# ORNL/DDStore

Hardware: NVIDIA H100
Metric: batch_fetch_GBps (higher is better)
Workload: dtype u8

## Files before the change

ddstore_b200/csrc/kernels.cu:

```cuda
#include <cuda_runtime.h>
#include <stdint.h>
#include <stdio.h>
#include <stdlib.h>
#include <string.h>

#include <algorithm>
#include <atomic>
#include <type_traits>

#include "kernels.h"

namespace {

thread_local char g_cuda_err[512] = "";
std::atomic<unsigned long long> g_launches{0};

#define CUDA_TRY(expr)                                                                                   \
    do {                                                                                                 \
        cudaError_t e__ = (expr);                                                                        \
        if (e__ != cudaSuccess) {                                                                        \
            snprintf(g_cuda_err, sizeof(g_cuda_err), "%s failed: %s (%s:%d)", #expr, cudaGetErrorString(e__), \
                     __FILE__, __LINE__);                                                                \
            return (int)e__ ? (int)e__ : -1;                                                             \
        }                                                                                                \
// ... 176 lines not shown
            start[k] = e.x;
            count[k] = e.y;
        }
    } else if (p.ids) {
        int64_t id[K];
#pragma unroll
        for (int k = 0; k < K; k++) {
            live[k] = idx[k] < limit;
            id[k] = live[k] ? p.ids[idx[k]] : 0;
            vp[k] = &var;
        }
#pragma unroll
        for (int k = 0; k < K; k++) {
            badid[k] = live[k] && (id[k] < 0 || id[k] >= p.nsamples);
            const bool ok = live[k] && !badid[k];
            const longlong2 e = ok ? ldg_pair(&p.tab[id[k]]) : make_longlong2(0, 0);
            start[k] = e.x;
            count[k] = e.y;
        }
    } else {
#pragma unroll
        for (int k = 0; k < K; k++) {
            live[k] = idx[k] < limit;
            badid[k] = false;
            start[k] = live[k] ? p.starts[idx[k]] : 0;
            count[k] = live[k] ? p.counts[idx[k]] : 0;
            vp[k] = &var;
        }
    }
#pragma unroll
    for (int k = 0; k < K; k++) {
        src[k] = 0;
        nbytes[k] = 0;
        if (!live[k]) continue;
        if (badid[k]) {
            report(status, tag, idx[k], DDSK_CODE_SAMPLE);
            continue;
        }
        uint64_t s = 0;
        const int code = dev_locate(*vp[k], start[k], count[k], &s);
        if (code) {
            report(status, tag, idx[k], code);
            continue;
        }
        src[k] = s;
        nbytes[k] = count[k] * vp[k]->row_bytes;
    }
}

__device__ __forceinline__ int64_t warp_incl_scan(int64_t v, int lane) {
#pragma unroll
    for (int d = 1; d < 32; d <<= 1) {
        int64_t o = __shfl_up_sync(0xffffffffu, v, d);
        if (lane >= d) v += o;
    }
    return v;
}
__device__ __forceinline__ int64_t warp_sum(int64_t v) {
#pragma unroll
    for (int d = 16; d > 0; d >>= 1) v += __shfl_xor_sync(0xffffffffu, v, d);
    return v;
}

struct GatherArgs {
    ddsk_var_t var;
    const int64_t *starts;
    int64_t count;
    const uint64_t *req_src;
    const int64_t *req_dst;
    const uint32_t *seg_tab;
    PlanSrc plan;
    int64_t *total_out;
    int64_t nreq;
    char *dst;
    int64_t dst_cap;
    int64_t *offsets_out;
    unsigned long long *status;
    unsigned long long status_tag;
    unsigned int *counters;
    char *mdst[DDSK_MAX_MULTI];
    int64_t mcap[DDSK_MAX_MULTI];
    int64_t *moffsets[DDSK_MAX_MULTI];
    int min_seg_chunks;
    int overlap, skip_wait;
    int wait1_valid, wait2_valid;
    unsigned int seq;
    unsigned int *ovl;
    int wait_plan;
    unsigned long long *plan_word;
    int64_t plan_tiles;
    unsigned int *tickets;
    unsigned long long *host_mirror;
    unsigned long long *dbg;
    const ddsk_push_t *push;
    int64_t push_nreq;
    unsigned long long push_step;
};

constexpr int64_t SEG_GRAIN = 16384;

struct Piece {
    uint64_t src;
    int64_t dpos;
    uint32_t n;
    uint32_t off;
};

template <int PCAP>
struct PlanView {
    uint32_t src_s, dst_s;
    __device__ __forceinline__ uint64_t s(int64_t i) const { return lds64(src_s + (uint32_t)i * 8u); }
    __device__ __forceinline__ int64_t d(int64_t i) const { return (int64_t)lds32(dst_s + (uint32_t)i * 4u); }
};
template <>
struct PlanView<0> {
    const uint64_t *src;
    const int64_t *dst;
    const uint32_t *seg_tab;
    __device__ __forceinline__ uint64_t s(int64_t i) const { return __ldcg(&src[i]); }
    __device__ __forceinline__ int64_t d(int64_t i) const { return __ldcg(&dst[i]); }
};

template <bool FIXED, int CH, int PCAP, bool VALIGN = false>
struct ChunkWalker {
    int64_t seg_pos = 0, seg_end = 0, T = 0, seg_bytes = 0, nseg = 0, nb = 0;
    int64_t gwarp = 0, nwarps = 1;
    bool first_claim = true, static_claims = false;
    int64_t cur_seg = 0;
    unsigned int pend = 0;
    bool armed = false;
    bool gate_ok = true;
    int64_t r = 0, win_base = -64;
    int64_t nreq = 0;
    int push_n = 0, push_me = 0, push_par = 0;
    const int64_t *push_rbase = nullptr;
    const uint64_t *push_win = nullptr;
    int64_t push_idx_off = 0;
    PlanView<PCAP> pv;
    bool valign = false;
    int64_t vb[VALIGN ? DDSK_MAX_MULTI : 1];
    uint64_t w_src = 0;
    int64_t w_dst = 0, w_n = 0;

    __device__ __forceinline__ void load_window(const GatherArgs &a, int lane) {
        win_base = r;
        int64_t idx = r + lane;
        w_src = 0;
        w_dst = 0;
        w_n = 0;
        if (idx < nreq) {
            if (FIXED && push_n > 0) {
                int p = 0;
                for (int k = 1; k < push_n; k++)
                    if (idx >= push_rbase[k]) p = k;
                const int64_t i = idx - push_rbase[p];
                const int64_t start = ld_relaxed_sys_s64((const int64_t *)(push_win[p] + push_idx_off) + i);
                uint64_t s = 0;
                int owner = 0;
                const int code = dev_locate_owner(a.var, start, a.count, &s, &owner);
                if (code && owner == push_me) {
                    unsigned long long *st = (unsigned long long *)push_win[p] + 3;
                    asm volatile("red.relaxed.sys.global.min.u64 [%0], %1;" ::"l"(st), "l"(((unsigned long long)i << 8) | (unsigned long long)code) : "memory");
                }
                w_src = (code || owner != push_me) ? 0 : s;
                w_dst = idx * nb;
                w_n = nb;
            } else if (FIXED) {
                uint64_t s = 0;
                int code = dev_locate(a.var, a.starts[idx], a.count, &s);
                if (code) report(a.status, a.status_tag, idx, code);
                w_src = code ? 0 : s;
                w_dst = idx * nb;
                w_n = nb;
            } else {
                w_src = pv.s(idx);
                w_dst = pv.d(idx);
                w_n = pv.d(idx + 1) - w_dst;
            }
        }
    }

    __device__ __forceinline__ int64_t align_to_var(int64_t pos) const {
        int64_t b = vb[0];
#pragma unroll
        for (int k = 1; k < (VALIGN ? DDSK_MAX_MULTI : 1); k++)
            if (pos >= vb[k]) b = vb[k];
        return b + ((pos - b) & ~(int64_t)7);
    }

    __device__ __forceinline__ int64_t locate_var(const GatherArgs &a, int64_t pos, int lane) {
        if constexpr (VALIGN && PCAP == 0) {
            if (valign) {
                int64_t r0 = (int64_t)__ldcg(&a.seg_tab[(pos + 7) / SEG_GRAIN]);
                while (r0 > 0 && pv.d(r0) > pos) r0--;
                return r0;
            }
        }
        if (PCAP == 0) {
            int64_t r0 = (int64_t)__ldcg(&a.seg_tab[pos / SEG_GRAIN]);
            return r0;
        }
        int64_t lo = 0, hi = nreq;
        while (hi - lo > 1) {
            int64_t step = (hi - lo + 31) / 32;
            int64_t idx = lo + (int64_t)(lane + 1) * step;
            bool le = (idx < hi) && (pv.d(idx) <= pos);
            int k = __popc(__ballot_sync(0xffffffffu, le));
            lo = lo + (int64_t)k * step;
            hi = min(hi, lo + step);
        }
        return lo;
    }

    __device__ __forceinline__ void arm(const GatherArgs &a, int lane) {
        if (lane == 0) pend = atomicAdd(a.tickets, 1u);
        armed = true;
    }

    template <int STAGE, typename Gate>
    __device__ __forceinline__ uint32_t next_group(const GatherArgs &a, int lane, Piece &pc, Gate &&gate) {
        while (true) {
            if (seg_pos >= seg_end) {
                int64_t seg;
                if (first_claim) {
                    first_claim = false;
                    seg = gwarp;
                    if (!static_claims && seg < nseg && gate_ok) arm(a, lane);
                } else if (static_claims) {
                    seg = cur_seg + nwarps;
                } else {
                    if (!armed) {
                        gate();
                        gate_ok = true;
                        arm(a, lane);
                    }
                    seg = nwarps + (int64_t)__shfl_sync(0xffffffffu, pend, 0);
                    armed = false;
                    if (seg < nseg) arm(a, lane);
                }
                cur_seg = seg;
                if (seg >= nseg) return 0;
                seg_pos = seg * seg_bytes;
                seg_end = min(T, seg_pos + seg_bytes);
                if constexpr (VALIGN) {
                    if (valign) {
                        seg_pos = align_to_var(seg_pos);
                        if (seg_end < T) seg_end = align_to_var(seg_end);
                        if (seg_pos >= seg_end) continue;
                    }
                }
                r = FIXED ? seg_pos / nb : locate_var(a, seg_pos, lane);
            }
            if (r >= nreq) {
                seg_pos = seg_end;
                continue;
            }
            if (r < win_base || r >= win_base + 32) load_window(a, lane);
            {
                const int wl = (int)(r - win_base);
                const uint64_t s0 = __shfl_sync(0xffffffffu, w_src, wl);
                const int64_t d0 = __shfl_sync(0xffffffffu, w_dst, wl);
                const int64_t e0 = d0 + __shfl_sync(0xffffffffu, w_n, wl);
                const int64_t p0 = max(d0, seg_pos);
                const int64_t len = min(min(e0, seg_end) - p0, (int64_t)CH);
                if (len >= CH / 2 || p0 + len < e0) {
                    seg_pos = p0 + len;
                    if (seg_pos >= e0) r++;
                    if (s0 == 0) continue;
                    const uint64_t src = s0 + (uint64_t)(p0 - d0);
                    pc.src = lane == 0 ? src : 0;
                    pc.dpos = p0;
                    pc.n = lane == 0 ? (uint32_t)len : 0u;
                    pc.off = 0;
                    return ((uint32_t)(src & 15u) + (uint32_t)len + 15u) & ~15u;
                }
            }
            const int srcl = (int)(r - win_base) + lane;
            const uint64_t q_src = __shfl_sync(0xffffffffu, w_src, srcl & 31);
            const int64_t q_d0 = __shfl_sync(0xffffffffu, w_dst, srcl & 31);
            const int64_t q_n = __shfl_sync(0xffffffffu, w_n, srcl & 31);
            const int64_t q_end = q_d0 + q_n;
            const bool valid = srcl < 32 && r + lane < nreq && q_d0 < seg_end;
            const int64_t p0 = max(q_d0, seg_pos);
            int64_t len = min(q_end, seg_end) - p0;
            len = max(len, (int64_t)0);
            len = min(len, (int64_t)CH);
            const bool complete = p0 + len >= q_end;
            const bool copy = valid && len > 0 && q_src != 0;
            const uint64_t src = q_src + (uint64_t)(p0 - q_d0);
            const uint32_t sz = copy ? (((uint32_t)(src & 15u) + (uint32_t)len + 15u) & ~15u) : 0u;
            uint32_t end = sz;
#pragma unroll
            for (int d = 1; d < 32; d <<= 1) {
                uint32_t o = __shfl_up_sync(0xffffffffu, end, d);
                if (lane >= d) end += o;
            }
            const unsigned ok = __ballot_sync(0xffffffffu, valid && end <= (uint32_t)STAGE);
            const unsigned part = __ballot_sync(0xffffffffu, valid && !complete);
            int m = ok == 0xffffffffu ? 32 : __ffs(~ok) - 1;
            if (part) m = min(m, __ffs(part));
            const bool active = lane < m;
            const int64_t new_pos = __shfl_sync(0xffffffffu, p0 + len, m - 1);
            const uint32_t total = __shfl_sync(0xffffffffu, end, m - 1);
            r += __popc(__ballot_sync(0xffffffffu, active && complete));
            seg_pos = max(seg_pos, new_pos);
            if (total == 0) continue;
            pc.src = (active && copy) ? src : 0;
            pc.dpos = p0;
            pc.n = (active && copy) ? (uint32_t)len : 0u;
            pc.off = end - sz;
            return total;
        }
    }
};

template <int WS, bool BYTES>
__device__ __forceinline__ void rephase_loop(uint32_t sbase, char *dv, uint32_t nv, uint32_t bs8, int lane) {
#pragma unroll 4
    for (uint32_t j = (uint32_t)lane; j < nv; j += 32) {
        const uint4 lo = lds128(sbase + (j << 4));
        const uint4 hi = lds128(sbase + (j << 4) + 16);
        const uint32_t w[8] = {lo.x, lo.y, lo.z, lo.w, hi.x, hi.y, hi.z, hi.w};
        uint4 out;
        if (BYTES) {
            out.x = __funnelshift_r(w[WS + 0], w[WS + 1], bs8);
            out.y = __funnelshift_r(w[WS + 1], w[WS + 2], bs8);
// ... 172 lines not shown
        const uint32_t k = head + nv * E + (uint32_t)lane;
        cvt_one<CODE>(s0 + (k << IL), d + ((size_t)k << OL), lut);
    }
}

struct NoCvt {
    int32_t unused_;
};
template <bool CVT>
using CvtParam = typename std::conditional<CVT, ddsk_cvt_t, NoCvt>::type;

template <int NW, int PCAP, bool CVT = false>
__device__ __forceinline__ int64_t plan_in_smem(const GatherArgs &a, const PlanView<PCAP> &pv, int64_t *wtot, int warp,
                                                int lane, bool writer, int code = 0) {
    auto out = [&](int64_t x) -> int64_t {
        if constexpr (CVT) return cvt_scale(x, code);
        else return x;
    };
    const int64_t nreq = a.nreq;
    const int64_t per_warp = ((nreq + NW * 128 - 1) / (NW * 128)) * 128;
    const int64_t w0 = min(nreq, (int64_t)warp * per_warp), w1 = min(nreq, w0 + per_warp);
    int64_t lane_sum = 0;
    for (int64_t b = w0; b < w1; b += 128) {
        int64_t idx[4], nb[4];
        uint64_t sv[4];
#pragma unroll
        for (int k = 0; k < 4; k++) idx[k] = b + k * 32 + lane;
        plan_many<4>(a.var, a.plan, idx, w1, a.status, a.status_tag, sv, nb);
#pragma unroll
        for (int k = 0; k < 4; k++) {
            if (idx[k] < w1) {
                sts64(pv.src_s + (uint32_t)idx[k] * 8u, sv[k]);
                sts32(pv.dst_s + (uint32_t)idx[k] * 4u, (uint32_t)min(nb[k], (int64_t)0xFFFFFFFFll));
                lane_sum += nb[k];
            }
        }
    }
    const int64_t wsum = warp_sum(lane_sum);
    if (lane == 0) wtot[warp] = wsum;
    __syncthreads();
    int64_t mine = lane < NW ? wtot[lane] : 0;
    const int64_t T = warp_sum(mine);
    const int64_t base = warp_sum(lane < warp ? mine : 0);
    int64_t run = base;
    for (int64_t b = w0; b < w1; b += 32) {
        const int64_t i = b + lane;
        const int64_t v = i < w1 ? (int64_t)lds32(pv.dst_s + (uint32_t)i * 4u) : 0;
        const int64_t incl = warp_incl_scan(v, lane);
        if (i < w1) {
            sts32(pv.dst_s + (uint32_t)i * 4u, (uint32_t)(run + incl - v));
            if (writer && a.offsets_out) a.offsets_out[i] = out(run + incl - v);
        }
        run += __shfl_sync(0xffffffffu, incl, 31);
    }
    if (warp == 0 && lane == 0) {
        sts32(pv.dst_s + (uint32_t)nreq * 4u, (uint32_t)min(T, (int64_t)0xFFFFFFFFll));
        if (writer) {
            if (a.offsets_out) a.offsets_out[nreq] = out(T);
            if (a.total_out) *a.total_out = T;
        }
    }
    __syncthreads();
    return T;
}

struct PieceDesc {
    int64_t dpos;
    uint32_t n, pack;
};

__device__ __forceinline__ void spin_until_done(const unsigned int *ovl, unsigned int q, unsigned long long *status,
                                                unsigned long long tag, int64_t nreq) {
    const uint64_t t0 = globaltimer_ns();
    while ((int)(ld_acquire_u32(&ovl[4 + (q & 3u)]) - q) < 0) {
        __nanosleep(100);
        if (globaltimer_ns() - t0 > 4000000000ull) {
            report(status, tag, nreq, DDSK_CODE_WATCHDOG);
            __trap();
        }
    }
}

template <bool FIXED, int NW, int S, int CH, int PCAP, bool CVT = false>
__global__ void __launch_bounds__(NW * 32, 1) dds_gather_kernel(const __grid_constant__ GatherArgs a,
                                                                const __grid_constant__ CvtParam<CVT> c) {
    constexpr int STAGE = CH + 32;
    constexpr bool PUSH = FIXED && !CVT;
    extern __shared__ __align__(128) unsigned char smem_dyn[];
    __shared__ __align__(8) uint64_t full_bar[NW][S];
    __shared__ __align__(16) PieceDesc desc[NW][S][32];
    __shared__ int64_t wtot[PCAP > 0 ? NW : 1];
    __shared__ int64_t push_rbase[PUSH ? DDSK_MAX_RANKS + 1 : 1];
    __shared__ uint64_t push_win[PUSH ? DDSK_MAX_RANKS : 1];

    const int lane = threadIdx.x & 31;
    const int warp = threadIdx.x >> 5;
    const int64_t gwarp = (int64_t)blockIdx.x * NW + warp;
    const int64_t nwarps = (int64_t)gridDim.x * NW;

    if (lane == 0) {
#pragma unroll
        for (int s = 0; s < S; s++) mbar_init(smem_u32(&full_bar[warp][s]), 1);
        fence_mbar_init();
    }
    uint32_t lut_s = 0;
    if constexpr (CVT) {
        lut_s = smem_u32(smem_dyn) + (uint32_t)(NW * S * STAGE + (PCAP ? PCAP * 12 + 16 : 0));
        for (int i = threadIdx.x; i < c.lut_bytes / 4; i += NW * 32) sts32(lut_s + 4u * (uint32_t)i, c.lut[i]);
        __syncthreads();
    }
    int code0 = 0;
    if constexpr (CVT) code0 = c.code[0];
    if (a.dbg && threadIdx.x == 0) a.dbg[blockIdx.x * 4 + 0] = globaltimer_ns();
    if (a.overlap && !a.wait1_valid) {
        asm volatile("griddepcontrol.wait;" ::: "memory");
        asm volatile("griddepcontrol.launch_dependents;" ::: "memory");
    } else {
        asm volatile("griddepcontrol.launch_dependents;" ::: "memory");
        if (!a.skip_wait) asm volatile("griddepcontrol.wait;" ::: "memory");
    }
    bool gate_open = !(a.overlap && a.wait2_valid);
    auto pass_gate = [&]() {
        if (!gate_open) {
            if (lane == 0) spin_until_done(a.ovl, a.seq - 2u, a.status, a.status_tag, a.nreq);
            __syncwarp();
            gate_open = true;
        }
    };

    ChunkWalker<FIXED, CH, PCAP, CVT> w;
    if (!FIXED) {
        if constexpr (PCAP > 0) {
            w.pv.src_s = smem_u32(smem_dyn) + (uint32_t)(NW * S * STAGE);
            w.pv.dst_s = w.pv.src_s + (uint32_t)PCAP * 8u;
            const bool writer = blockIdx.x == 0;
            if (writer) pass_gate();
            w.T = plan_in_smem<NW, PCAP, CVT>(a, w.pv, wtot, warp, lane, writer, code0);
        } else {
            w.pv.src = a.req_src;
            w.pv.dst = a.req_dst;
            w.pv.seg_tab = a.seg_tab;
            if (a.wait_plan) {
                const bool need_gate = !gate_open;
                unsigned long long pw = 0;
                const uint64_t t0 = globaltimer_ns();
                while (true) {
                    bool ok = true;
                    if (lane == 0) {
                        pw = ld_acquire_u64(&a.plan_word[a.seq & 3u]);
                        ok = (pw >> 40) == (unsigned long long)a.plan_tiles;
                    } else if (lane == 1 && need_gate) {
                        ok = (int)(ld_acquire_u32(&a.ovl[4 + ((a.seq - 2u) & 3u)]) - (a.seq - 2u)) >= 0;
                    }
                    if (__all_sync(0xffffffffu, ok)) break;
                    __nanosleep(100);
                    if (globaltimer_ns() - t0 > 4000000000ull) {
                        report(a.status, a.status_tag, a.nreq, DDSK_CODE_WATCHDOG);
                        __trap();
                    }
                }
                gate_open = true;
                w.T = (int64_t)(__shfl_sync(0xffffffffu, pw, 0) & 0xFFFFFFFFFFull);
            } else {
                w.T = __ldcg(&a.req_dst[a.nreq]);
            }
        }
    }

    const bool push = PUSH && a.push != nullptr;
    if (FIXED && push) {
        const ddsk_push_t *ps = a.push;
        const int P = ps->nranks, me = ps->me, par = (int)(a.push_step & 1ull);
        if (blockIdx.x == 0 && threadIdx.x == 0) {
            unsigned long long *hdr = (unsigned long long *)ps->win[me];
            *(volatile unsigned long long *)&hdr[1 + par] = (unsigned long long)a.push_nreq;
            __threadfence_system();
            st_release_sys_u64(&hdr[0], a.push_step);
        }
        const uint64_t t0 = globaltimer_ns();
        for (int r0 = 0; r0 < P; r0 += 32) {
            const int r = r0 + lane;
            while (r < P && ld_acquire_sys_u64((const unsigned long long *)ps->win[r]) < a.push_step) {
                __nanosleep(200);
                if (globaltimer_ns() - t0 > 30000000000ull) {
                    report(a.status, a.status_tag, a.nreq, DDSK_CODE_WATCHDOG);
                    __trap();
                }
            }
        }
        __syncwarp();
        if (warp == 0) {
            int64_t n = 0;
            for (int r0 = 0; r0 < P; r0 += 32) {
                const int r = r0 + lane;
                int64_t mine_n = 0;
                if (r < P) {
                    push_win[r] = (uint64_t)ps->win[r];
                    mine_n = ld_relaxed_sys_s64((const int64_t *)ps->win[r] + 1 + par);
                }
                const int64_t incl = warp_incl_scan(mine_n, lane);
                if (r < P) push_rbase[r] = n + incl - mine_n;
                n += __shfl_sync(0xffffffffu, incl, 31);
            }
            if (lane == 0) push_rbase[P] = n;
        }
        __syncthreads();
        w.push_n = P;
        w.push_me = me;
        w.push_par = par;
        w.push_rbase = push_rbase;
        w.push_win = push_win;
        w.push_idx_off = ps->idx_off[par];
    }
    if (a.dbg && threadIdx.x == 0) a.dbg[blockIdx.x * 4 + 1] = globaltimer_ns();
    bool dbg_first = a.dbg != nullptr && warp == 0;
    w.gwarp = gwarp;
    w.nwarps = nwarps;
    w.static_claims = a.tickets == nullptr;
    w.gate_ok = gate_open;
    w.nb = (FIXED && a.count <= a.var.lenlist[a.var.nranks - 1]) ? a.count * a.var.row_bytes : 0;
    w.nreq = (FIXED && push) ? push_rbase[w.push_n] : a.nreq;
    if (FIXED) w.T = w.nb * w.nreq;
    bool over = w.T > a.dst_cap;
    const int64_t push_dst_off = (FIXED && push) ? a.push->dst_off[w.push_par] : 0;
    const bool multi = !FIXED && a.plan.nvars > 1;
    int64_t vbase[DDSK_MAX_MULTI + 1];
#pragma unroll
    for (int v = 0; v <= DDSK_MAX_MULTI; v++) vbase[v] = INT64_MAX;
    if (multi) {
        over = false;
#pragma unroll
        for (int v = 0; v < DDSK_MAX_MULTI; v++)
            if (v < a.plan.nvars) vbase[v] = w.pv.d((int64_t)v * a.plan.per_var);
#pragma unroll
        for (int v = 0; v < DDSK_MAX_MULTI; v++)
            if (v < a.plan.nvars) {
                const int64_t endv = v + 1 < a.plan.nvars ? vbase[v + 1] : w.T;
                over |= endv - vbase[v] > a.mcap[v];
            }
        if (PCAP > 0) over |= w.T > 0xFFFFFFFFll;
        if constexpr (CVT) {
            w.valign = true;
#pragma unroll
            for (int v = 0; v < DDSK_MAX_MULTI; v++) w.vb[v] = vbase[v];
        }
    }
    auto dst_of = [&](int64_t dpos) -> char * {
        if (FIXED && push) {
            int p = 0;
            for (int k = 1; k < w.push_n; k++)
                if (dpos >= push_rbase[k] * w.nb) p = k;
            return (char *)push_win[p] + push_dst_off + (dpos - push_rbase[p] * w.nb);
        }
        if (!multi) return a.dst + dpos;
        int64_t b = vbase[0];
        char *d = a.mdst[0];
#pragma unroll
        for (int k = 1; k < DDSK_MAX_MULTI; k++)
            if (dpos >= vbase[k]) {
                b = vbase[k];
                d = a.mdst[k];
            }
        return d + (dpos - b);
    };
    auto out_of = [&](int64_t dpos, int &code, uint32_t &lut) -> char * {
        if constexpr (CVT) {
            if (!multi) {
                code = code0;
                lut = lut_s + (uint32_t)c.lut_off[0];
                return a.dst + cvt_scale(dpos, code0);
            }
            int64_t b = vbase[0];
            char *d = a.mdst[0];
            int cd = c.code[0], lo = c.lut_off[0];
#pragma unroll
            for (int k = 1; k < DDSK_MAX_MULTI; k++)
                if (dpos >= vbase[k]) {
                    b = vbase[k];
                    d = a.mdst[k];
                    cd = c.code[k];
                    lo = c.lut_off[k];
                }
            code = cd;
            lut = lut_s + (uint32_t)lo;
            return d + cvt_scale(dpos - b, cd);
        } else {
            return nullptr;
        }
    };
    {
        int64_t target = w.T / (nwarps * 8);
        const int64_t unit = (!FIXED && PCAP == 0) ? SEG_GRAIN : (int64_t)CH;
        target = max((int64_t)a.min_seg_chunks * CH, min(target, (int64_t)1 << 20));
        target = max(target, unit);
        if (FIXED && w.nb > 0 && w.nb <= target)
            w.seg_bytes = (target / w.nb) * w.nb;
        else
            w.seg_bytes = (target / unit) * unit;
        w.nseg = w.T > 0 ? (w.T + w.seg_bytes - 1) / w.seg_bytes : 0;
    }
    if (over) {
        if (gwarp == 0 && lane == 0) report(a.status, a.status_tag, a.nreq, DDSK_CODE_CAPACITY);
        w.nseg = 0;
    }

    if (FIXED && !push && (w.nb <= 0 || over)) {
        for (int64_t i = gwarp * 32 + lane; i < a.nreq; i += nwarps * 32) {
            uint64_t s;
            int code = dev_locate(a.var, a.starts[i], a.count, &s);
            if (code) report(a.status, a.status_tag, i, code);
        }
    }

    const uint32_t ring = smem_u32(smem_dyn) + (uint32_t)warp * (uint32_t)(S * STAGE);

    uint32_t issued = 0, consumed = 0;
    bool more = w.nseg > 0;
    while (true) {
        while (more && issued - consumed < (uint32_t)(S - 1)) {
            Piece pc;
            const uint32_t total = w.template next_group<STAGE>(a, lane, pc, pass_gate);
            if (total == 0) {
                more = false;
                break;
            }
            const uint32_t st = issued % S;
            const uint32_t bar = smem_u32(&full_bar[warp][st]);
            bulk_wait_read<1>();
            if (lane == 0) mbar_expect_tx(bar, total);
            __syncwarp();
            const uint32_t al = (uint32_t)(pc.src & 15u);
            desc[warp][st][lane].dpos = pc.dpos;
            desc[warp][st][lane].n = pc.n;
            desc[warp][st][lane].pack = pc.off | (al << 16);
            if (pc.n)
                tma_load_1d(ring + st * STAGE + pc.off, (const void *)(pc.src - al), (al + pc.n + 15u) & ~15u, bar);
            issued++;
        }
        if (consumed == issued) break;
        const uint32_t st = consumed % S;
        const uint32_t parity = (consumed / S) & 1u;
        const uint32_t bar = smem_u32(&full_bar[warp][st]);
        if (!mbar_try_wait(bar, parity)) {
            const uint64_t t0 = globaltimer_ns();
            while (!mbar_try_wait(bar, parity)) {
                if (globaltimer_ns() - t0 > 4000000000ull) {
                    report(a.status, a.status_tag, a.nreq, DDSK_CODE_WATCHDOG);
                    __trap();
                }
            }
        }
        __syncwarp();
        if (dbg_first) {
            dbg_first = false;
            if (lane == 0) a.dbg[blockIdx.x * 4 + 2] = globaltimer_ns();
        }
        pass_gate();
        if (!w.static_claims && !w.gate_ok) {
            w.gate_ok = true;
            if (!w.armed) w.arm(a, lane);
        }
        const int64_t my_dpos = desc[warp][st][lane].dpos;
        const uint32_t my_n = desc[warp][st][lane].n;
        const uint32_t my_pack = desc[warp][st][lane].pack;
        if constexpr (CVT) {
            int my_code;
            uint32_t my_lut;
            char *const my_dst = out_of(my_dpos, my_code, my_lut);
            const bool direct = my_code == 0 && my_n != 0 && (((uint32_t)(uint64_t)my_dst | my_n | (my_pack >> 16)) & 15u) == 0;
            if (direct) tma_store_1d(my_dst, ring + st * STAGE + (my_pack & 0xffffu), my_n);
            unsigned todo = __ballot_sync(0xffffffffu, my_n != 0 && !direct);
            while (todo) {
                const int j = __ffs(todo) - 1;
                todo &= todo - 1;
                const int64_t dpos = __shfl_sync(0xffffffffu, my_dpos, j);
                const uint32_t n = __shfl_sync(0xffffffffu, my_n, j);
                const uint32_t pk = __shfl_sync(0xffffffffu, my_pack, j);
                int code;
                uint32_t lut;
                char *const d = out_of(dpos, code, lut);
                const uint32_t s0 = ring + st * STAGE + (pk & 0xffffu);
                switch (code) {
                case DDSK_CVT_F32_BF16: cvt_drain<DDSK_CVT_F32_BF16>(s0 + (pk >> 16), d, n, lut, lane); break;
                case DDSK_CVT_F32_F16: cvt_drain<DDSK_CVT_F32_F16>(s0 + (pk >> 16), d, n, lut, lane); break;
                case DDSK_CVT_F64_F32: cvt_drain<DDSK_CVT_F64_F32>(s0 + (pk >> 16), d, n, lut, lane); break;
                case DDSK_CVT_U8_LUT16: cvt_drain<DDSK_CVT_U8_LUT16>(s0 + (pk >> 16), d, n, lut, lane); break;
                case DDSK_CVT_U8_LUT32: cvt_drain<DDSK_CVT_U8_LUT32>(s0 + (pk >> 16), d, n, lut, lane); break;
                default: drain_chunk<CH>(s0, pk >> 16, d, n, lane); break;
                }
            }
        } else {
        char *const my_dst = dst_of(my_dpos);
        const bool direct = my_n != 0 && (((uint32_t)(uint64_t)my_dst | my_n | (my_pack >> 16)) & 15u) == 0;
        if (direct) tma_store_1d(my_dst, ring + st * STAGE + (my_pack & 0xffffu), my_n);
        unsigned todo = __ballot_sync(0xffffffffu, my_n != 0 && !direct);
        while (todo) {
            const int j = __ffs(todo) - 1;
            todo &= todo - 1;
            const int64_t dpos = __shfl_sync(0xffffffffu, my_dpos, j);
            const uint32_t n = __shfl_sync(0xffffffffu, my_n, j);
            const uint32_t pk = __shfl_sync(0xffffffffu, my_pack, j);
            drain_chunk<CH>(ring + st * STAGE + (pk & 0xffffu), pk >> 16, dst_of(dpos), n, lane);
        }
        }
        bulk_commit();
        __syncwarp();
        consumed++;
    }
    if (a.overlap || (FIXED && push)) {
        bulk_wait_all<0>();
        fence_proxy_async_global();
    } else {
        bulk_wait_read<0>();
    }
    __syncwarp();
    pass_gate();
    if (multi) {
        for (int64_t i = gwarp * 32 + lane; i < a.nreq + a.plan.nvars; i += nwarps * 32) {
            const int v = (int)(i / (a.plan.per_var + 1));
            const int64_t j = i - (int64_t)v * (a.plan.per_var + 1);
            if (v < a.plan.nvars && a.moffsets[v]) {
                const int64_t basev = w.pv.d((int64_t)v * a.plan.per_var);
                int64_t e = (v * a.plan.per_var + j == a.nreq) ? w.T : w.pv.d((int64_t)v * a.plan.per_var + j);
                if constexpr (CVT) a.moffsets[v][j] = cvt_scale(e - basev, c.code[v]);
                else a.moffsets[v][j] = e - basev;
            }
        }
        if constexpr (CVT) {
            if (gwarp == 0 && lane == 0 && a.total_out) {
                int64_t t = 0;
#pragma unroll
                for (int v = 0; v < DDSK_MAX_MULTI; v++)
                    if (v < a.plan.nvars) t += cvt_scale((v + 1 < a.plan.nvars ? vbase[v + 1] : w.T) - vbase[v], c.code[v]);
                *a.total_out = t;
            }
        }
    }
    if (FIXED && a.offsets_out && !push) {
        if constexpr (CVT) {
            for (int64_t i = gwarp * 32 + lane; i <= a.nreq; i += nwarps * 32) a.offsets_out[i] = cvt_scale(i * w.nb, code0);
        } else {
            for (int64_t i = gwarp * 32 + lane; i <= a.nreq; i += nwarps * 32) a.offsets_out[i] = i * w.nb;
        }
// ... 260 lines not shown
        __syncthreads();
        const int state = sh_state;
        const unsigned long long q = req[0];
        if (state != 0) {
            if (threadIdx.x == 0) {
                if (state == 2) {
                    *(volatile unsigned long long *)&mb->resp = (q << 8);
                    __threadfence_system();
                }
                *(volatile unsigned long long *)&mb->exit_gen = gen;
                __threadfence_system();
            }
            return;
        }
        const int64_t start = (int64_t)req[1], count = (int64_t)req[2], cap = (int64_t)req[4];
        char *dp = (char *)req[3];
        const ddsk_var_t &var = vars[(int)(req[5] & 0xFFFFFFFFull)];
        uint64_t src = 0;
        const int code = dev_locate(var, start, count, &src);
        const int64_t n = code ? 0 : count * var.row_bytes;
        unsigned long long st = 0;
        if (code) st = (unsigned long long)code;
        else if (n > cap) st = DDSK_CODE_CAPACITY;
        if (st == 0 && n > 0) {
            const char *sp = (const char *)src;
            if ((((uint64_t)sp | (uint64_t)dp | (uint64_t)n) & 15u) == 0) {
                for (int64_t i = threadIdx.x; i < (n >> 4); i += blockDim.x) ((uint4 *)dp)[i] = ((const uint4 *)sp)[i];
            } else if ((((uint64_t)sp | (uint64_t)dp | (uint64_t)n) & 3u) == 0) {
                for (int64_t i = threadIdx.x; i < (n >> 2); i += blockDim.x) ((uint32_t *)dp)[i] = ((const uint32_t *)sp)[i];
            } else {
                for (int64_t i = threadIdx.x; i < n; i += blockDim.x) dp[i] = sp[i];
            }
            __threadfence_system();
        }
        __syncthreads();
        if (threadIdx.x == 0) *(volatile unsigned long long *)&mb->resp = (q << 8) | st;
        served = q;
    }
}

__global__ void dds_touch_kernel(const uint4 *__restrict__ p, size_t n, unsigned int *sink) {
    unsigned int acc = 0;
    for (size_t i = (size_t)blockIdx.x * blockDim.x + threadIdx.x; i < n; i += (size_t)gridDim.x * blockDim.x) {
        const uint4 v = p[i];
        acc ^= v.x ^ v.y ^ v.z ^ v.w;
    }
    if (acc == 0x9E3779B9u && sink) *sink = acc;
}

__global__ void dds_occupy_kernel(unsigned long long ns, int smem_bytes) {
    extern __shared__ unsigned char occ_smem[];
    if ((int)threadIdx.x < smem_bytes) occ_smem[threadIdx.x] = (unsigned char)threadIdx.x;
    const uint64_t t0 = globaltimer_ns();
    while (globaltimer_ns() - t0 < ns) __nanosleep(1000);
    if ((int)threadIdx.x < smem_bytes && occ_smem[threadIdx.x] == 255 && ns == 0) printf("");
}

struct Geometry {
    int nw, stages, ch, pcap;
};
constexpr Geometry kGeoms[] = {{8, 4, 4096, 0}, {8, 6, 4096, 0}, {16, 3, 4096, 0}, {4, 4, 8192, 0}, {12, 4, 4096, 0}, {4, 6, 4096, 0},
                               {6, 4, 4096, 0},
                               {12, 3, 4096, 0}};
constexpr int kNumGeoms = (int)(sizeof(kGeoms) / sizeof(kGeoms[0]));
constexpr Geometry kGeomsS[] = {{12, 3, 4096, 4096}, {12, 3, 3072, 8192}, {16, 3, 2048, 8192}, {16, 3, 3072, 4096}, {8, 4, 4096, 4096}};
constexpr int kNumGeomsS = (int)(sizeof(kGeomsS) / sizeof(kGeomsS[0]));
constexpr int64_t kPlanSmemMax = 8192;
int64_t g_plan_smem_default = 1024;

constexpr int kGeomLarge = 4, kGeomSmall = 2, kGeomVar = 4;

int g_geom_fixed_env = -1;
int g_geom_var_env = -1;
int g_geom_s_env = -1;
int g_min_seg_var = 4, g_min_seg_s = 2;
bool g_geom_init = false;
int g_sms = 0;
int g_ctas_per_sm = 1;
int g_pdl = 1;
unsigned long long *g_dbg = nullptr;
constexpr size_t kDbgRegion = 4096 + 8;
int g_l2_persist = 1;
int g_smem_plan = 1;

int pick_geometry() {
    if (g_geom_init) return 0;
    int dev = 0;
    CUDA_TRY(cudaGetDevice(&dev));
    CUDA_TRY(cudaDeviceGetAttribute(&g_sms, cudaDevAttrMultiProcessorCount, dev));
    if (const char *e = getenv("DDS_GATHER_GEOM")) g_geom_fixed_env = atoi(e);
    if (g_geom_fixed_env >= kNumGeoms) g_geom_fixed_env = -1;
    g_geom_var_env = g_geom_fixed_env;
    if (const char *e = getenv("DDS_GATHER_GEOM_VAR")) g_geom_var_env = atoi(e);
    if (g_geom_var_env >= kNumGeoms) g_geom_var_env = -1;
    if (const char *e = getenv("DDS_GATHER_GEOM_S")) g_geom_s_env = atoi(e);
    if (g_geom_s_env >= kNumGeomsS) g_geom_s_env = -1;
    if (const char *e = getenv("DDS_VAR_MINSEG")) g_min_seg_var = atoi(e) > 0 ? atoi(e) : 4;
    if (const char *e = getenv("DDS_S_MINSEG")) g_min_seg_s = atoi(e) > 0 ? atoi(e) : 2;
    if (const char *e = getenv("DDS_GATHER_CTAS_PER_SM")) g_ctas_per_sm = atoi(e) > 0 ? atoi(e) : 1;
    if (const char *e = getenv("DDS_PDL")) g_pdl = atoi(e) != 0;
    if (const char *e = getenv("DDS_SMEM_PLAN")) g_smem_plan = atoi(e);
    if (const char *e = getenv("DDS_SMEM_PLAN_MAX")) g_plan_smem_default = atoll(e);
    if (const char *e = getenv("DDS_L2_PERSIST")) g_l2_persist = atoi(e);
    if (const char *e = getenv("DDS_DEBUG_TIMING"))
        if (atoi(e)) {
            CUDA_TRY(cudaMalloc((void **)&g_dbg, 2 * kDbgRegion * 8));
            CUDA_TRY(cudaMemset(g_dbg, 0, 2 * kDbgRegion * 8));
        }
    g_geom_init = true;
    return 0;
}

int geometry_for(bool fixed, int64_t request_bytes) {
    if (fixed) {
        if (g_geom_fixed_env >= 0) return g_geom_fixed_env;
        return request_bytes < 2048 ? kGeomSmall : kGeomLarge;
    }
    return g_geom_var_env >= 0 ? g_geom_var_env : kGeomVar;
}
int geometry_s_for(int64_t nreq) {
    if (nreq > kPlanSmemMax || nreq > g_plan_smem_default) return -1;
    if (g_geom_s_env >= 0 && kGeomsS[g_geom_s_env].pcap >= nreq) return g_geom_s_env;
    return nreq <= 4096 ? 0 : 1;
}

constexpr int smem_bytes_of(int nw, int s, int ch, int pcap) { return nw * s * (ch + 32) + (pcap ? pcap * 12 + 16 : 0); }
int static_smem_of(int nw, int s) { return nw * s * (8 + 32 * 16) + 16 * 8 + 64; }
int ctas_per_sm_for(int nw, int s, int ch, int pcap) {
    int per_sm = g_ctas_per_sm;
    while (per_sm > 1 && per_sm * (smem_bytes_of(nw, s, ch, pcap) + static_smem_of(nw, s) + 1024) > 227 * 1024) per_sm--;
    return per_sm;
}

template <bool FIXED, int NW, int S, int CH, int PCAP, bool CVT = false>
int launch_gather_t(const GatherArgs &args_in, cudaStream_t stream, const ddsk_cvt_t *cvt = nullptr) {
    const int smem = smem_bytes_of(NW, S, CH, PCAP) + (CVT ? cvt->lut_bytes : 0);
    static std::atomic<unsigned long long> configured{0};
    auto kern = dds_gather_kernel<FIXED, NW, S, CH, PCAP, CVT>;
    int dev = 0;
    CUDA_TRY(cudaGetDevice(&dev));
    if (CVT) {
        if (dev >= 64 || !(configured.load() & (1ull << dev))) {
            cudaFuncAttributes fa;
            int optin = 0;
            CUDA_TRY(cudaFuncGetAttributes(&fa, kern));
            CUDA_TRY(cudaDeviceGetAttribute(&optin, cudaDevAttrMaxSharedMemoryPerBlockOptin, dev));
            const int most = std::min(smem_bytes_of(NW, S, CH, PCAP) + DDSK_MAX_MULTI * 1024, optin - (int)fa.sharedSizeBytes);
            CUDA_TRY(cudaFuncSetAttribute(kern, cudaFuncAttributeMaxDynamicSharedMemorySize, most));
            if (dev < 64) configured.fetch_or(1ull << dev);
        }
    } else if (dev >= 64 || !(configured.load() & (1ull << dev))) {
        CUDA_TRY(cudaFuncSetAttribute(kern, cudaFuncAttributeMaxDynamicSharedMemorySize, smem));
        if (dev < 64) configured.fetch_or(1ull << dev);
    }
    const int per_sm = ctas_per_sm_for(NW, S, CH, PCAP);
    GatherArgs args = args_in;
    args.dbg = g_dbg ? g_dbg + (size_t)(args.overlap ? (args.seq & 1u) : 0u) * kDbgRegion : nullptr;
    cudaLaunchConfig_t cfg = {};
    cfg.gridDim = dim3((unsigned)(g_sms * per_sm));
    cfg.blockDim = dim3(NW * 32);
    cfg.dynamicSmemBytes = smem;
    cfg.stream = stream;
    cudaLaunchAttribute attr[1];
    attr[0].id = cudaLaunchAttributeProgrammaticStreamSerialization;
    attr[0].val.programmaticStreamSerializationAllowed = g_pdl ? 1 : 0;
    cfg.attrs = attr;
    cfg.numAttrs = 1;
    if constexpr (CVT) {
        CUDA_TRY(cudaLaunchKernelEx(&cfg, kern, args, *cvt));
    } else {
        CUDA_TRY(cudaLaunchKernelEx(&cfg, kern, args, NoCvt{0}));
    }
    g_launches++;
    return 0;
}

template <int NW, int S, int CH, int PCAP>
bool cvt_s_fits_t(int lut_bytes) {
    cudaFuncAttributes fa;
    int dev = 0, optin = 0;
    if (cudaGetDevice(&dev) != cudaSuccess || cudaFuncGetAttributes(&fa, dds_gather_kernel<false, NW, S, CH, PCAP, true>) != cudaSuccess ||
        cudaDeviceGetAttribute(&optin, cudaDevAttrMaxSharedMemoryPerBlockOptin, dev) != cudaSuccess) {
        (void)cudaGetLastError();
        return false;
    }
    return smem_bytes_of(NW, S, CH, PCAP) + lut_bytes + (int)fa.sharedSizeBytes <= optin;
}

thread_local const void *g_l2_base = nullptr;
thread_local size_t g_l2_bytes = 0;

template <typename... KArgs, typename... Args>
int launch_pdl(void (*kern)(KArgs...), dim3 grid, dim3 block, cudaStream_t st, Args... args) {
    cudaLaunchConfig_t cfg = {};
    cfg.gridDim = grid;
    cfg.blockDim = block;
    cfg.dynamicSmemBytes = 0;
    cfg.stream = st;
    cudaLaunchAttribute attr[2];
    attr[0].id = cudaLaunchAttributeProgrammaticStreamSerialization;
    attr[0].val.programmaticStreamSerializationAllowed = g_pdl ? 1 : 0;
    cfg.attrs = attr;
    cfg.numAttrs = 1;
    if (g_l2_base && g_l2_bytes && g_l2_persist) {
        attr[1].id = cudaLaunchAttributeAccessPolicyWindow;
        attr[1].val.accessPolicyWindow.base_ptr = const_cast<void *>(g_l2_base);
        attr[1].val.accessPolicyWindow.num_bytes = g_l2_bytes;
        attr[1].val.accessPolicyWindow.hitRatio = 1.0f;
        attr[1].val.accessPolicyWindow.hitProp = cudaAccessPropertyPersisting;
        attr[1].val.accessPolicyWindow.missProp = cudaAccessPropertyStreaming;
        cfg.numAttrs = 2;
    }
    g_l2_base = nullptr;
    g_l2_bytes = 0;
    CUDA_TRY(cudaLaunchKernelEx(&cfg, kern, args...));
    g_launches++;
    return 0;
}

template <bool FIXED>
int launch_gather(const GatherArgs &args, cudaStream_t stream, const ddsk_cvt_t *cvt) {
    if (cvt) return launch_gather_t<FIXED, 12, 4, 4096, 0, true>(args, stream, cvt);
    const int64_t request_bytes = args.count < ((int64_t)1 << 20) ? args.count * args.var.row_bytes : INT64_MAX;
    switch (geometry_for(FIXED, FIXED ? request_bytes : 0)) {
    case 1: return launch_gather_t<FIXED, 8, 6, 4096, 0>(args, stream);
    case 2: return launch_gather_t<FIXED, 16, 3, 4096, 0>(args, stream);
    case 3: return launch_gather_t<FIXED, 4, 4, 8192, 0>(args, stream);
    case 4: return launch_gather_t<FIXED, 12, 4, 4096, 0>(args, stream);
    case 5: return launch_gather_t<FIXED, 4, 6, 4096, 0>(args, stream);
    case 6: return launch_gather_t<FIXED, 6, 4, 4096, 0>(args, stream);
    case 7: return launch_gather_t<FIXED, 12, 3, 4096, 0>(args, stream);
    default: return launch_gather_t<FIXED, 8, 4, 4096, 0>(args, stream);
    }
}
int launch_gather_s(int g, const GatherArgs &args, cudaStream_t stream, const ddsk_cvt_t *cvt) {
    if (cvt) return g == 1 ? launch_gather_t<false, 12, 3, 3072, 8192, true>(args, stream, cvt)
                           : launch_gather_t<false, 12, 3, 4096, 4096, true>(args, stream, cvt);
    switch (g) {
    case 1: return launch_gather_t<false, 12, 3, 3072, 8192>(args, stream);
    case 2: return launch_gather_t<false, 16, 3, 2048, 8192>(args, stream);
    case 3: return launch_gather_t<false, 16, 3, 3072, 4096>(args, stream);
    case 4: return launch_gather_t<false, 8, 4, 4096, 4096>(args, stream);
    default: return launch_gather_t<false, 12, 3, 4096, 4096>(args, stream);
    }
}

int select_s(int64_t nreq, int64_t cap, const ddsk_cvt_t *cvt) {
    if (!g_smem_plan || cap >= ((int64_t)1 << 32)) return -1;
    if (!cvt) return geometry_s_for(nreq);
    if (nreq > kPlanSmemMax || nreq > g_plan_smem_default) return -1;
    if (nreq <= 4096) return cvt_s_fits_t<12, 3, 4096, 4096>(cvt->lut_bytes) ? 0 : -1;
    return cvt_s_fits_t<12, 3, 3072, 8192>(cvt->lut_bytes) ? 1 : -1;
}

void fill_overlap(GatherArgs &a, const ddsk_scratch_t *scr, int flags) {
    a.overlap = (flags & DDSK_F_OVERLAP) ? 1 : 0;
    a.skip_wait = (flags & DDSK_F_SKIP_WAIT) ? 1 : 0;
    a.wait1_valid = (flags & DDSK_F_PREV1) ? 1 : 0;
    a.wait2_valid = (flags & DDSK_F_PREV2) ? 1 : 0;
    a.seq = scr->ovl_seq;
    a.ovl = scr->ovl;
    a.tickets = a.overlap ? nullptr : scr->counters;
}

}

extern "C" {

const char *ddsk_last_cuda_error(void) { return g_cuda_err; }
unsigned long long ddsk_launch_count(void) { return g_launches.load(); }
int64_t ddsk_plan_smem_max(void) { return kPlanSmemMax; }
int ddsk_debug_timing(unsigned long long *host_out, int max_words) {
    if (!g_dbg) return 0;
    const size_t n = (size_t)max_words < 2 * kDbgRegion ? (size_t)max_words : 2 * kDbgRegion;
    if (cudaMemcpy(host_out, g_dbg, n * 8, cudaMemcpyDeviceToHost) != cudaSuccess) return -1;
    return (int)n;
}

void ddsk_gather_geometry(int *ctas, int *warps_per_cta, int *stages, int *chunk_bytes, int *smem_bytes) {
    if (pick_geometry()) {
        *ctas = *warps_per_cta = *stages = *chunk_bytes = *smem_bytes = 0;
        return;
    }
    const Geometry &g = kGeoms[geometry_for(true, 4096)];
    *ctas = g_sms * ctas_per_sm_for(g.nw, g.stages, g.ch, 0);
    *warps_per_cta = g.nw;
    *stages = g.stages;
    *chunk_bytes = g.ch;
    *smem_bytes = smem_bytes_of(g.nw, g.stages, g.ch, 0);
}

int ddsk_gather_fixed(const ddsk_var_t *var, const int64_t *starts_dev, int64_t count, int64_t nreq, void *dst_dev,
                      int64_t dst_capacity, int64_t *offsets_dev_or_null, const ddsk_scratch_t *scr, int flags,
                      const ddsk_cvt_t *cvt, void *stream) {
    cudaStream_t st = (cudaStream_t)stream;
    if (flags & DDSK_F_RESET) CUDA_TRY(cudaMemsetAsync(scr->status, 0xFF, sizeof(unsigned long long), st));
    if (nreq <= 0) return 0;
    if (int rc = pick_geometry()) return rc;
    GatherArgs a;
    memset(&a, 0, sizeof(a));
    a.var = *var;
    a.starts = starts_dev;
    a.count = count;
    a.nreq = nreq;
    a.dst = (char *)dst_dev;
    a.dst_cap = dst_capacity;
    a.offsets_out = offsets_dev_or_null;
    a.status = scr->status;
    a.status_tag = scr->status_tag;
    a.counters = scr->counters;
    a.min_seg_chunks = 1;
    fill_overlap(a, scr, flags);
    a.host_mirror = (flags & DDSK_F_MIRROR) ? scr->host_mirror : nullptr;
    return launch_gather<true>(a, st, cvt);
}

int ddsk_gather_push(const ddsk_var_t *var, const ddsk_push_t *push_host, const ddsk_push_t *push_dev,
                     const int64_t *starts_dev, int64_t count, int64_t nreq, unsigned long long step,
                     const ddsk_scratch_t *scr, void *stream) {
    cudaStream_t st = (cudaStream_t)stream;
    if (int rc = pick_geometry()) return rc;
    GatherArgs a;
    memset(&a, 0, sizeof(a));
    a.var = *var;
    a.count = count;
    a.nreq = nreq;
    a.dst = nullptr;
    a.dst_cap = INT64_MAX;
    a.status = scr->status;
    a.status_tag = scr->status_tag;
    a.counters = scr->counters;
    a.tickets = scr->counters;
    a.min_seg_chunks = 1;
    a.push = push_dev;
    if (nreq > 0)
        CUDA_TRY(cudaMemcpyAsync(push_host->win[push_host->me] + push_host->idx_off[step & 1ull], starts_dev, (size_t)nreq * 8,
                                 cudaMemcpyDeviceToDevice, st));
    a.push_nreq = nreq;
    a.push_step = step;
    return launch_gather<true>(a, st, nullptr);
}

static int plan_and_gather(const ddsk_var_t *var, const PlanSrc &p, int64_t nreq, int64_t cap_total, GatherArgs &a,
                           int64_t *offsets_dev_or_null, ddsk_scratch_t *scr, int flags, const ddsk_cvt_t *cvt,
                           cudaStream_t st) {
// ... 199 lines not shown
```

Measured before the change: 1440.

## Add tail-splitting segment scheduler and bound gather kernel registers

Adds an optional segment scheduler, enabled by DDS_SEG_SCHED and off by default, that keeps bulk segments on static or ticket claims. The remaining tail is split into progressively smaller chunks tracked in per-warp shared state, to reduce load imbalance at the end of a gather. It also changes variable-length request lookup to a bounded warp binary search between seg_tab entries, replacing the valign backtracking. Separately, it swaps __launch_bounds__(NW*32,1) for __maxnreg__(128), which changes register allocation and occupancy on the default path and may add spills.

```diff
diff --git a/ddstore_b200/csrc/kernels.cu b/ddstore_b200/csrc/kernels.cu
--- a/ddstore_b200/csrc/kernels.cu
+++ b/ddstore_b200/csrc/kernels.cu
@@ -282,6 +282,7 @@
     int64_t mcap[DDSK_MAX_MULTI];
     int64_t *moffsets[DDSK_MAX_MULTI];
     int min_seg_chunks;
+    int seg_sched;
     int overlap, skip_wait;
     int wait1_valid, wait2_valid;
     unsigned int seq;
@@ -325,8 +326,11 @@
 struct ChunkWalker {
     int64_t seg_pos = 0, seg_end = 0, T = 0, seg_bytes = 0, nseg = 0, nb = 0;
     int64_t gwarp = 0, nwarps = 1;
-    bool first_claim = true, static_claims = false;
+    bool first_claim = true;
     int64_t cur_seg = 0;
+    int64_t nbulk = 0;
+    enum { FIRST = 0, N = 4, BASE = 8, REM = 12, S = 16, UNIT = 20 };
+    uint32_t tail_st = 0;
     unsigned int pend = 0;
     bool armed = false;
     bool gate_ok = true;
@@ -389,18 +393,13 @@
     }
 
     __device__ __forceinline__ int64_t locate_var(const GatherArgs &a, int64_t pos, int lane) {
-        if constexpr (VALIGN && PCAP == 0) {
-            if (valign) {
-                int64_t r0 = (int64_t)__ldcg(&a.seg_tab[(pos + 7) / SEG_GRAIN]);
-                while (r0 > 0 && pv.d(r0) > pos) r0--;
-                return r0;
-            }
-        }
+        int64_t lo = 0, hi = nreq;
         if (PCAP == 0) {
-            int64_t r0 = (int64_t)__ldcg(&a.seg_tab[pos / SEG_GRAIN]);
-            return r0;
-        }
-        int64_t lo = 0, hi = nreq;
+            const int64_t g = pos / SEG_GRAIN;
+            lo = (int64_t)__ldcg(&a.seg_tab[g]);
+            if (pos == g * SEG_GRAIN) return lo;
+            if ((g + 1) * SEG_GRAIN < T) hi = min(hi, (int64_t)__ldcg(&a.seg_tab[g + 1]) + 1);
+        }
         while (hi - lo > 1) {
             int64_t step = (hi - lo + 31) / 32;
             int64_t idx = lo + (int64_t)(lane + 1) * step;
@@ -415,6 +414,41 @@
     __device__ __forceinline__ void arm(const GatherArgs &a, int lane) {
         if (lane == 0) pend = atomicAdd(a.tickets, 1u);
         armed = true;
+    }
+
+    __device__ __forceinline__ static bool stride(const GatherArgs &a) { return FIXED && a.overlap; }
+    __device__ __forceinline__ bool ticket_next(const GatherArgs &a) const {
+        return a.tickets != nullptr && (!stride(a) || cur_seg + nwarps >= nbulk);
+    }
+
+    __device__ __forceinline__ void set_round(uint32_t first, uint32_t base, uint32_t rem) {
+        const uint32_t s = max(1u, rem / (2u * (uint32_t)nwarps));
+        sts32(tail_st + FIRST, first);
+        sts32(tail_st + N, min((uint32_t)nwarps, rem / s));
+        sts32(tail_st + BASE, base);
+        sts32(tail_st + REM, rem);
+        sts32(tail_st + S, s);
+    }
+    __device__ __forceinline__ void start_tail(uint32_t smem, int64_t unit) {
+        tail_st = smem;
+        const int64_t tail0 = nbulk * seg_bytes;
+        sts32(tail_st + UNIT, (uint32_t)unit);
+        set_round(0, 0, T > tail0 ? (uint32_t)((T - tail0 + unit - 1) / unit) : 0u);
+    }
+    __device__ __forceinline__ bool tail_claim(int64_t j) {
+        if (nbulk == nseg) return false;
+        uint32_t first = lds32(tail_st + FIRST), n = lds32(tail_st + N);
+        while (j >= (int64_t)first + n) {
+            if (n == 0) return false;
+            const uint32_t s = lds32(tail_st + S);
+            set_round(first + n, lds32(tail_st + BASE) + n * s, lds32(tail_st + REM) - n * s);
+            first = lds32(tail_st + FIRST);
+            n = lds32(tail_st + N);
+        }
+        const uint32_t s = lds32(tail_st + S), unit = lds32(tail_st + UNIT);
+        seg_pos = nbulk * seg_bytes + (int64_t)(lds32(tail_st + BASE) + ((uint32_t)j - first) * s) * unit;
+        seg_end = min(T, seg_pos + (int64_t)s * unit);
+        return true;
     }
 
     template <int STAGE, typename Gate>
@@ -425,8 +459,7 @@
                 if (first_claim) {
                     first_claim = false;
                     seg = gwarp;
-                    if (!static_claims && seg < nseg && gate_ok) arm(a, lane);
-                } else if (static_claims) {
+                } else if (a.tickets == nullptr || (stride(a) && cur_seg + nwarps < nbulk)) {
                     seg = cur_seg + nwarps;
                 } else {
                     if (!armed) {
@@ -434,14 +467,17 @@
                         gate_ok = true;
                         arm(a, lane);
                     }
-                    seg = nwarps + (int64_t)__shfl_sync(0xffffffffu, pend, 0);
+                    seg = (stride(a) ? max(nbulk, nwarps) : nwarps) + (int64_t)__shfl_sync(0xffffffffu, pend, 0);
                     armed = false;
-                    if (seg < nseg) arm(a, lane);
                 }
                 cur_seg = seg;
-                if (seg >= nseg) return 0;
-                seg_pos = seg * seg_bytes;
-                seg_end = min(T, seg_pos + seg_bytes);
+                if (seg < nbulk) {
+                    seg_pos = seg * seg_bytes;
+                    seg_end = min(T, seg_pos + seg_bytes);
+                } else if (!tail_claim(seg - nbulk)) {
+                    return 0;
+                }
+                if (gate_ok && !armed && ticket_next(a)) arm(a, lane);
                 if constexpr (VALIGN) {
                     if (valign) {
                         seg_pos = align_to_var(seg_pos);
@@ -780,7 +816,7 @@
 }
 
 template <bool FIXED, int NW, int S, int CH, int PCAP, bool CVT = false>
-__global__ void __launch_bounds__(NW * 32, 1) dds_gather_kernel(const __grid_constant__ GatherArgs a,
+__global__ void __maxnreg__(128) dds_gather_kernel(const __grid_constant__ GatherArgs a,
                                                                 const __grid_constant__ CvtParam<CVT> c) {
     constexpr int STAGE = CH + 32;
     constexpr bool PUSH = FIXED && !CVT;
@@ -790,6 +826,7 @@
     __shared__ int64_t wtot[PCAP > 0 ? NW : 1];
     __shared__ int64_t push_rbase[PUSH ? DDSK_MAX_RANKS + 1 : 1];
     __shared__ uint64_t push_win[PUSH ? DDSK_MAX_RANKS : 1];
+    __shared__ uint32_t tail_st[NW][6];
 
     const int lane = threadIdx.x & 31;
     const int warp = threadIdx.x >> 5;
@@ -914,7 +951,6 @@
     bool dbg_first = a.dbg != nullptr && warp == 0;
     w.gwarp = gwarp;
     w.nwarps = nwarps;
-    w.static_claims = a.tickets == nullptr;
     w.gate_ok = gate_open;
     w.nb = (FIXED && a.count <= a.var.lenlist[a.var.nranks - 1]) ? a.count * a.var.row_bytes : 0;
     w.nreq = (FIXED && push) ? push_rbase[w.push_n] : a.nreq;
@@ -1001,6 +1037,11 @@
         if (gwarp == 0 && lane == 0) report(a.status, a.status_tag, a.nreq, DDSK_CODE_CAPACITY);
         w.nseg = 0;
     }
+    w.nbulk = w.nseg;
+    if (a.seg_sched && !(FIXED && push) && w.nseg > 0) {
+        w.nbulk = w.stride(a) ? max(w.nseg / nwarps - 1, (int64_t)0) * nwarps : max(w.nseg - nwarps, (int64_t)0);
+        w.start_tail(smem_u32(&tail_st[warp][0]), (FIXED && w.nb <= w.seg_bytes) ? (CH + w.nb - 1) / w.nb * w.nb : (int64_t)CH);
+    }
 
     if (FIXED && !push && (w.nb <= 0 || over)) {
         for (int64_t i = gwarp * 32 + lane; i < a.nreq; i += nwarps * 32) {
@@ -1054,9 +1095,9 @@
             if (lane == 0) a.dbg[blockIdx.x * 4 + 2] = globaltimer_ns();
         }
         pass_gate();
-        if (!w.static_claims && !w.gate_ok) {
+        if (a.tickets != nullptr && !w.gate_ok) {
             w.gate_ok = true;
-            if (!w.armed) w.arm(a, lane);
+            if (!w.armed && w.ticket_next(a)) w.arm(a, lane);
         }
         const int64_t my_dpos = desc[warp][st][lane].dpos;
         const uint32_t my_n = desc[warp][st][lane].n;
@@ -1483,6 +1524,7 @@
 constexpr size_t kDbgRegion = 4096 + 8;
 int g_l2_persist = 1;
 int g_smem_plan = 1;
+int g_seg_sched = 0;
 
 int pick_geometry() {
     if (g_geom_init) return 0;
@@ -1503,6 +1545,7 @@
     if (const char *e = getenv("DDS_SMEM_PLAN")) g_smem_plan = atoi(e);
     if (const char *e = getenv("DDS_SMEM_PLAN_MAX")) g_plan_smem_default = atoll(e);
     if (const char *e = getenv("DDS_L2_PERSIST")) g_l2_persist = atoi(e);
+    if (const char *e = getenv("DDS_SEG_SCHED")) g_seg_sched = atoi(e) != 0;
     if (const char *e = getenv("DDS_DEBUG_TIMING"))
         if (atoi(e)) {
             CUDA_TRY(cudaMalloc((void **)&g_dbg, 2 * kDbgRegion * 8));
@@ -1661,7 +1704,8 @@
     a.wait2_valid = (flags & DDSK_F_PREV2) ? 1 : 0;
     a.seq = scr->ovl_seq;
     a.ovl = scr->ovl;
-    a.tickets = a.overlap ? nullptr : scr->counters;
+    a.seg_sched = g_seg_sched;
+    a.tickets = !a.overlap ? scr->counters : g_seg_sched ? scr->ovl + 8 + (a.seq & 3u) : nullptr;
 }
 
 }
```

Result: no change. 1440, median of 6 (-0.0%).
